# Chunyu-Hugh/SymbolicRegression.jl

Hardware: AMD Instinct MI355X
Metric: tree-node x row evals/sec (batched eval_loss, fp32) (higher is better)
Workload: dtype f32

## Files before the change

symbolicregression.jl_amd/csrc/sr_capi.cpp:

```cpp
#include <hip/hip_runtime.h>
#include <rccl/rccl.h>
#include <dlfcn.h>
#include <limits.h>
#include <stdlib.h>

#include <algorithm>
#include <atomic>
#include <chrono>
#include <cmath>
#include <cstdio>
#include <cstdlib>
#include <cstring>
#include <deque>
#include <functional>
#include <memory>
#include <mutex>
#include <string>
#include <vector>

#include "../../include/sr_amd.h"
#include "sr_compile.h"
#include "sr_eval.h"
#include "sr_fold.h"
#include "sr_fold_dev.h"
// ... 864 lines not shown
    prog->max_depth = 0;
    prog->tier = tier;
    prog->max_checks = 0;
    prog->total_nodes = 0;
    prog->total_ops = 0;
    hprog = ctx->h_prog.as<char>();
    h_code = reinterpret_cast<SrIns<T>*>(hprog);
    h_off = reinterpret_cast<uint32_t*>(hprog + img.o_off);
    h_bad = reinterpret_cast<uint8_t*>(hprog + img.o_bad);
    h_perm = reinterpret_cast<uint32_t*>(hprog + img.o_perm);
    ctx->h_bad_last = h_bad;
    ctx->h_perm_last = h_perm;
    h_end = reinterpret_cast<uint32_t*>(hprog + img.o_end);
    last.n_chunks = 0;
    last.derived = false;
    last.n_derived = 0;
    last.timed = ctx->timing != 0 && !want.internal;
    if (last.timed) SR_HIP_CHECK(hipEventRecord(ctx->ev_start, s));
    if (gather)
      SR_HIP_CHECK(hipMemcpyAsync(ctx->row_idx.p, req.row_idx, size_t(n_rows_up) * sizeof(int64_t), hipMemcpyHostToDevice,
                                  s));
    if (parametric && nt > 0 && p_stride > 0)
      SR_HIP_CHECK(hipMemcpyAsync(ctx->ptab.p, ctx->h_ptab.p, size_t(nt) * size_t(p_stride) * sizeof(T), hipMemcpyHostToDevice, s));
    return SR_OK;
  }

  int launch_derived() {
    dld = (n_eval + kRowAlign - 1) / kRowAlign * kRowAlign;
    max_abs_x = leaf_bound(want.shard ? want.shard->max_abs_x : req.ds->max_abs_x);
    const int64_t derived_rows = want.shard ? want.shard->min_rows : n_eval;
    if (allow_derived && ctx->derived && want.mode == SR_MODE_LOSS && tier == SR_TIER_BASIC &&
        derived_rows >= kDerivedMinRows && nt >= 64 && double(nt) * double(derived_rows) >= kDerivedMinWork &&
        max_abs_x < double(tbig())) {
      choose_derived(*req.trees, ctx->opsets[req.opset_id], req.ds->nf, &spec, &dmap);
      if (spec.n > 0) {
        SR_HIP_CHECK(ctx->derived_cols.ensure(size_t(spec.n) * size_t(dld) * sizeof(T)));
        if (last.timed) SR_HIP_CHECK(hipEventRecord(ctx->ev_d0, s));
        SR_HIP_CHECK(sr_launch_derived<T>(static_cast<const T*>(req.ds->X), req.ds->ld,
                                          gather ? ctx->row_idx.as<int64_t>() : nullptr, n_eval, dld, spec,
                                          ctx->derived_cols.as<T>(), dld, s));
        if (last.timed) SR_HIP_CHECK(hipEventRecord(ctx->ev_d1, s));
        last.derived = true;
        last.n_derived = spec.n;
      } else {
        dmap.clear();
      }
    }
    stress_probe = use_probe && !gather && req.ds->probe_rows != nullptr && ctx->stress_probe;
    if (stress_probe && !dmap.empty()) {
      SR_HIP_CHECK(ctx->probe_derived.ensure(size_t(spec.n) * size_t(kProbeRows) * sizeof(T)));
      SR_HIP_CHECK(sr_launch_derived<T>(static_cast<const T*>(req.ds->X), req.ds->ld,
                                        static_cast<const int64_t*>(req.ds->probe_rows), req.ds->n_probe, kProbeRows, spec,
                                        ctx->probe_derived.as<T>(), kProbeRows, s));
    }
    return SR_OK;
  }

  int begin_chunks() {
    if (n_chunks > 1) {
      SR_HIP_CHECK(ctx->need_stream2());
      SR_HIP_CHECK(hipEventRecord(ctx->ev_join, s));
      SR_HIP_CHECK(hipStreamWaitEvent(ctx->stream2, ctx->ev_join, 0));
    }
    fjob.path = fold.path;
    fjob.tier = tier;
    fjob.gather = gather;
    fjob.n_eval = n_eval;
// ... 3452 lines not shown
```

symbolicregression.jl_amd/csrc/sr_compile.cpp:

```cpp
#include "sr_compile.h"

#include <unistd.h>

#include <algorithm>
#include <atomic>
#include <chrono>
#include <cstdlib>
#include <cmath>
#include <condition_variable>
#include <cstring>
#include <functional>
#include <mutex>
#include <thread>

namespace {

class WorkerPool {
 public:
  static WorkerPool& get() {
    static std::mutex m;
    static WorkerPool* pool = nullptr;
    std::lock_guard<std::mutex> g(m);
    if (!pool || pool->pid_ != getpid()) pool = new WorkerPool();
    return *pool;
// ... 129 lines not shown
  std::vector<T> fold_val;
  std::vector<int32_t> const_slot;
  std::vector<int32_t> need;
  std::vector<SrIns<T>> code;
  std::vector<int32_t> sz;
  bool bad = false;
  int err = SR_OK;
  std::string msg;
  int depth = 0, max_depth = 0;
  uint32_t n_checks = 0;
  uint32_t n_consts = 0;
  int64_t n_ops = 0;

  const int16_t* derived = nullptr;
  int max_params = 0;
  const bool fuse_pbc = [] {
    static const bool on = [] {
      const char* v = std::getenv("SR_AMD_PBC");
      return !(v && v[0] == '0');
    }();
    return on;
  }();

  TreeCompiler(const SrOpset& o, int64_t nr, int64_t nf, bool wci, const int16_t* dm = nullptr)
      : ops(o), n_rows(nr), nfeatures(nf), with_const_index(wci), derived(dm) {}

  int derived_col(int i) {
    if (!derived || t.degree[i] != 1) return -1;
    const int c = t.l[i];
    if (t.degree[c] != 0 || t.constant[c] || par(c)) return -1;
    const uint32_t u = unary_id(i);
    if (u == SR_U_NONE || u >= SR_U_COUNT) return -1;
    return derived[size_t(u) * size_t(nfeatures) + size_t(t.feature[c] - 1)];
  }

  bool leaf(int i) const { return t.degree[i] == 0; }
  bool par(int i) const { return t.is_param != nullptr && t.is_param[i] != 0; }
  bool effleaf(int i) const { return t.degree[i] == 0 || folded[i]; }

  uint32_t unary_id(int i) {
    const int k = int(t.op[i]) - 1;
    if (k < 0 || k >= int(ops.unary.size())) {
      fail(SR_ERR_BAD_TREE, "unary op index out of range");
      return SR_U_NONE;
    }
    return ops.unary[k];
  }
  uint32_t binary_id(int i) {
    const int k = int(t.op[i]) - 1;
    if (k < 0 || k >= int(ops.binary.size())) {
      fail(SR_ERR_BAD_TREE, "binary op index out of range");
      return SR_B_NONE;
    }
    return ops.binary[k];
  }
  void fail(int code, const char* m) {
    if (err == SR_OK) {
      err = code;
      msg = m;
    }
  }

  bool parse() {
    const int64_t n = t.n;
    if (n <= 0) {
      fail(SR_ERR_BAD_TREE, "empty tree");
// ... 270 lines not shown
    const bool free_c = base == SR_OP_LOAD_FEAT || base == SR_OP_LOAD_FEAT_PUSH ||
                        (base >= SR_OP_UNARY0 && base < SR_OP_LOAD_DERIVED) ||
                        (base >= SR_OP_BINARY0 && base < SR_OP_LOAD_PARAM && (base - SR_OP_BINARY0) % 6u < SR_V_CL) ||
                        (base >= SR_OP_LOAD_PARAM && base < SR_OP_PAIR0);
    if (!free_c) return false;
    uint32_t v = 0;
    switch (bop) {
      case SR_B_ADD: v = SR_PBC_ADD; break;
      case SR_B_SUB: v = left ? SR_PBC_SUB_L : SR_PBC_SUB_R; break;
      case SR_B_MUL: v = SR_PBC_MUL; break;
      case SR_B_DIV: v = left ? SR_PBC_DIV_L : SR_PBC_DIV_R; break;
      default: return false;
    }
    const_operand_check(leaf);
    last.op |= v << SR_OP_PBC_SHIFT;
    last.c0 = lf.c0;
    last.c1 = lf.c1;
    if (arr_check[i]) {
      last.op |= SR_OP_PBC_CHECK;
      ++n_checks;
    }
    return true;
  }

  void emit(int i) {
    if (effleaf(i)) {
      code.push_back(leaf_ins(i));
      emit_check(i);
      return;
    }
    const int d = t.degree[i];
    ++n_ops;
    if (d == 1) {
      const int dc = infsub[i] ? -1 : derived_col(i);
      if (dc >= 0) {
        SrIns<T> in{};
        in.op = SR_OP_LOAD_DERIVED;
        in.meta = uint32_t(dc);
        in.c0 = (unary_id(i) << 16) | uint32_t(t.feature[t.l[i]] - 1);
        code.push_back(in);
        emit_check(i);
        return;
      }
      emit(t.l[i]);
      if (!with_const_index && !code.empty() && (code.back().op >> SR_OP_POST_SHIFT) == 0u) {
        code.back().op |= (unary_id(i) << SR_OP_POST_SHIFT) | (infsub[i] ? SR_OP_POST_INF : 0u);
        if (arr_check[i]) {
          code.back().op |= SR_OP_POST_CHECK;
          ++n_checks;
        }
        return;
      }
      SrIns<T> in{};
      in.op = (infsub[i] ? SR_OP_UNARY_INF0 : SR_OP_UNARY0) + unary_id(i);
      code.push_back(in);
      emit_check(i);
      return;
    }
    const int a = t.l[i], b = t.r[i];
    const uint32_t bop = binary_id(i);
    if (err != SR_OK) return;
    if (emit_pair(i, bop)) {
    } else if (effleaf(b) && !(!with_const_index && par(b) && effleaf(a) && !par(a))) {
      emit(a);
      if (fuse_const_operand(i, b, bop, false)) return;
      const_operand_check(b);
// ... 294 lines not shown
```

symbolicregression.jl_amd/csrc/sr_compile.h:

```cpp
#pragma once
#include <stdint.h>
#include <functional>
#include <string>
#include <vector>
#include "sr_ops.h"
#include "../../include/sr_amd.h"

struct SrOpset {
  std::vector<uint32_t> unary;
  std::vector<uint32_t> binary;
};

uint32_t sr_unary_id(const char* name);
uint32_t sr_binary_id(const char* name);

template <typename T>
struct SrProgramBatch {
  std::vector<SrIns<T>> code;
  std::vector<uint32_t> offsets;
  std::vector<uint8_t> static_bad;
  std::vector<uint32_t> n_checks;
  std::vector<uint32_t> n_consts;
  std::vector<uint32_t> const_off;
  std::vector<uint32_t> cost;
  std::vector<uint8_t> depth;
  int max_depth = 0;
  int tier = 1;
  int max_checks = 0;
  int64_t total_nodes = 0;
  int64_t total_ops = 0;
  bool keep_pieces = false;
  std::vector<std::vector<SrIns<T>>> pieces;
  std::vector<uint32_t> piece, begin;
  size_t n_code = 0;
  const SrIns<T>* tree_code(size_t k) const {
    return keep_pieces ? pieces[piece[k]].data() + begin[k] : code.data() + offsets[k];
  }
};

void sr_parallel_for(int n, const std::function<void(int)>& fn);

uint32_t sr_instruction_cost(uint32_t opcode);

struct SrParamNodes {
  const uint8_t* is_parameter;
  const uint16_t* parameter;
  int32_t max_parameters;
};
template <typename T>
int sr_compile_batch(const sr_tree_batch& trees, const SrOpset& ops, int64_t n_rows, int64_t nfeatures,
                     bool with_const_index, SrProgramBatch<T>* out, std::string* err,
                     const int16_t* derived = nullptr, const SrParamNodes* pn = nullptr);
```

symbolicregression.jl_amd/csrc/sr_knobs.h:

```cpp
#pragma once
#include <stdint.h>
#include <stdlib.h>
#include <string.h>

#include <string>

#include "sr_plan.h"

struct SrKnobs {
  int tail_chunk = 4;
  int exact_early = 1;
  int64_t fold_seg = -1;
  int64_t host_reduce = 8192;
  int host_io = 1;
  int debug_hint_regrow = 0;
  int exact_g = 0;
  int exact_w = 4;
  int derived = 1;
  int stress_probe = 1;
  int code_cache = 1;
  int vstk_rows = 0;
  int grad_rows_force = 0;
  int grad_sort = 1;
  int grad_lane_bins = 1;
  int first_chunk = 6;
  int64_t chunk_min = 1024;
  int inject_fail = 0;
  int inject_post = 0;
  int inject_post_exact = 0;
  int inject_post_gather = 0;
  int inject_post_wsum = 0;
  int timing = 1;
  int rows_override = 0;
  int tree_group = 0;
  int waves_override = 0;
  bool cost_order = true;
  bool balance_groups = true;
  bool dead_hints = true;
  int max_row_blocks = 512;
  int chunks = 2;
  int probe = 2;
  int ref_fold = 1;
  int64_t fold_store_mb = 512;
  int64_t fold_slot_mb = 24576;
  int fold_delta_log2 = 8;
  int64_t fold_seg_max = 16384;
  int64_t fold_rows_max = int64_t(1) << 24;
  int fold_debug_fail = 0;
  int fold_single_pass = 1;
  int fold_compact = 1;
  int64_t fold_list_wgs = 2048;
// ... 9 lines not shown
struct SrKnobRow {
  const char* name;
  const char* env;
  int SrKnobs::*i32;
  int64_t SrKnobs::*i64;
  bool SrKnobs::*flag;
  SrKnobNorm norm;
  int64_t lo, hi;
  const char* refuse;
  bool env_inverse;

  constexpr SrKnobRow(const char* n, const char* e, int SrKnobs::*m, SrKnobNorm nm = SR_KNOB_RANGE, int64_t l = INT64_MIN,
                      int64_t h = INT64_MAX, const char* r = nullptr)
      : name(n), env(e), i32(m), i64(nullptr), flag(nullptr), norm(nm), lo(l), hi(h), refuse(r), env_inverse(false) {}
  constexpr SrKnobRow(const char* n, const char* e, int64_t SrKnobs::*m, int64_t l = INT64_MIN, int64_t h = INT64_MAX)
      : name(n), env(e), i32(nullptr), i64(m), flag(nullptr), norm(SR_KNOB_RANGE), lo(l), hi(h), refuse(nullptr),
        env_inverse(false) {}
  constexpr SrKnobRow(const char* n, const char* e, bool SrKnobs::*m, bool inverse = false)
      : name(n), env(e), i32(nullptr), i64(nullptr), flag(m), norm(SR_KNOB_FLAG), lo(0), hi(1), refuse(nullptr),
        env_inverse(inverse) {}
};

constexpr int64_t kKnobMax = INT64_MAX;

constexpr SrKnobRow kSrKnobs[] = {
    {"rows_per_lane", "SR_AMD_ROWS_PER_LANE", &SrKnobs::rows_override},
    {"trees_per_block", "SR_AMD_TREES_PER_BLOCK", &SrKnobs::tree_group, SR_KNOB_RANGE, 0, 256,
     "trees_per_block: 0, or 1..256 (4 waves of 64 slots)"},
    {nullptr, "SR_AMD_WAVES", &SrKnobs::waves_override},
    {"vstk_rows", "SR_AMD_VSTK_ROWS", &SrKnobs::vstk_rows},
    {"max_row_blocks", "SR_AMD_MAX_ROW_BLOCKS", &SrKnobs::max_row_blocks, SR_KNOB_RANGE, 1, 1 << 16},
    {"code_cache", "SR_AMD_CODE_CACHE", &SrKnobs::code_cache, SR_KNOB_FLAG},
    {"derived", "SR_AMD_DERIVED", &SrKnobs::derived, SR_KNOB_FLAG},
    {nullptr, "SR_AMD_NO_SORT", &SrKnobs::cost_order, true},
    {"balance", "SR_AMD_BALANCE", &SrKnobs::balance_groups},
    {nullptr, "SR_AMD_NO_HINT", &SrKnobs::dead_hints, true},
    {"probe", "SR_AMD_PROBE", &SrKnobs::probe},
    {"stress_probe", "SR_AMD_STRESS_PROBE", &SrKnobs::stress_probe, SR_KNOB_FLAG},
    {nullptr, "SR_AMD_CHUNKS", &SrKnobs::chunks},
    {"first_chunk", "SR_AMD_FIRST_CHUNK", &SrKnobs::first_chunk, SR_KNOB_RANGE, 2, 64},
    {"chunk_min", "SR_AMD_CHUNK_MIN", &SrKnobs::chunk_min, 1, kKnobMax},
    {"tail_chunk", "SR_AMD_TAIL_CHUNK", &SrKnobs::tail_chunk, SR_KNOB_RANGE, 0, kTailTwelfths,
     "tail_chunk: 0, or the last chunk's twelfths 1..6"},
    {"host_io", "SR_AMD_HOST_IO", &SrKnobs::host_io, SR_KNOB_RANGE, 0, 1, "host_io must be 0 or 1"},
    {"host_reduce", "SR_AMD_HOST_REDUCE", &SrKnobs::host_reduce, 0, kKnobMax},
    {"timing", nullptr, &SrKnobs::timing, SR_KNOB_FLAG},
    {"exact_g", "SR_AMD_EXACT_G", &SrKnobs::exact_g, SR_KNOB_RANGE, 0, 64},
    {"exact_w", "SR_AMD_EXACT_W", &SrKnobs::exact_w, SR_KNOB_EXACT_W},
    {"exact_early", "SR_AMD_EXACT_EARLY", &SrKnobs::exact_early, SR_KNOB_FLAG},
    {"grad_rows", "SR_AMD_GRAD_ROWS", &SrKnobs::grad_rows_force},
    {"grad_sort", "SR_AMD_GRAD_SORT", &SrKnobs::grad_sort, SR_KNOB_FLAG},
    {"grad_lane_bins", nullptr, &SrKnobs::grad_lane_bins, SR_KNOB_FLAG},
    {"ref_fold", "SR_AMD_REF_FOLD", &SrKnobs::ref_fold, SR_KNOB_FLAG},
    {"fold_seg", "SR_AMD_FOLD_SEG", &SrKnobs::fold_seg, -1, kKnobMax},
    {"fold_store_mb", "SR_AMD_FOLD_STORE_MB", &SrKnobs::fold_store_mb, 0, kKnobMax},
    {"fold_slot_mb", "SR_AMD_FOLD_SLOT_MB", &SrKnobs::fold_slot_mb, 1, kKnobMax},
    {"fold_delta_log2", "SR_AMD_FOLD_DELTA_LOG2", &SrKnobs::fold_delta_log2, SR_KNOB_RANGE, 1, 40},
    {"fold_seg_max", "SR_AMD_FOLD_SEG_MAX", &SrKnobs::fold_seg_max, 0, kKnobMax},
    {"fold_rows_max", "SR_AMD_FOLD_ROWS_MAX", &SrKnobs::fold_rows_max, 0, kKnobMax},
    {"fold_single_pass", "SR_AMD_FOLD_SINGLE_PASS", &SrKnobs::fold_single_pass, SR_KNOB_FLAG},
    {"fold_compact", "SR_AMD_FOLD_COMPACT", &SrKnobs::fold_compact, SR_KNOB_FLAG},
    {"fold_list_wgs", "SR_AMD_FOLD_LIST_WGS", &SrKnobs::fold_list_wgs, 0, kFoldListWgsMax},
    {"loss_compact", "SR_AMD_LOSS_COMPACT", &SrKnobs::loss_compact, SR_KNOB_FLAG},
    {"loss_list_groups", "SR_AMD_LOSS_LIST_GROUPS", &SrKnobs::loss_list_groups, SR_KNOB_RANGE, 0, 1 << 20},
    {"fold_cand_est", "SR_AMD_FOLD_CAND_EST", &SrKnobs::fold_cand_est, SR_KNOB_FLAG},
    {"fold_cand_est_min", "SR_AMD_FOLD_CAND_EST_MIN", &SrKnobs::fold_cand_est_min, SR_KNOB_RANGE, 1, 1 << 30},
// ... 43 lines not shown
```

symbolicregression.jl_amd/csrc/sr_plan.h:

```cpp
#pragma once
#include <stddef.h>
#include <stdint.h>

#include <algorithm>
#include <utility>
#include <vector>

#include "sr_compile.h"
#include "../../include/sr_amd.h"

enum { SR_MODE_LOSS = 0, SR_MODE_PRED = 1, SR_MODE_EXACT = 2, SR_MODE_FOLD = 3 };
#ifndef SR_VSTK_SLOTS
#define SR_VSTK_SLOTS 2
#endif
enum { SR_TIER_BASIC = 0, SR_TIER_FULL = 1 };
enum { SR_TIER_PARAM = 2 };
enum { SR_TIER_CAND = 4 };

struct SrSegment {
  int block0, pos0, n_pos, groups;
  int64_t row_off;
};

constexpr int SR_MAX_DERIVED = 32;
struct SrDerivedSpec {
  int n;
  uint8_t op[SR_MAX_DERIVED];
  uint16_t feat[SR_MAX_DERIVED];
};

template <typename T>
inline int sr_rows_per_lane(int mode, int tier, int requested) {
  const bool basic = mode == SR_MODE_LOSS && tier == SR_TIER_BASIC;
  if (sizeof(T) == 4) {
    if (basic) return (requested == 4 || requested == 16) ? requested : 8;
    return 4;
  }
  return basic ? 4 : 2;
}

inline size_t sr_tile_lds_bytes(int elem_size, int nf, int rows_per_lane, int stack_depth, int trees_per_block,
                                int max_checks, int waves, bool weighted, int code_lds = 0) {
  const size_t rows = size_t(64) * rows_per_lane;
  return size_t(nf) * rows * elem_size + (weighted ? 2 : 1) * rows * elem_size +
         size_t(waves) * stack_depth * rows * elem_size + size_t(waves) * size_t(max_checks) * rows * elem_size +
         (size_t(trees_per_block) * size_t(max_checks) * elem_size + 15) / 16 * 16 + size_t(code_lds) * 16;
}

inline int sr_waves_per_block(int elem_size, int mode, int tier, int rows_per_lane, int requested) {
  if (elem_size == 4 && mode == SR_MODE_LOSS && tier == SR_TIER_BASIC && rows_per_lane == 8 && requested == 8)
    return 8;
  return 4;
}

#ifndef SR_VSTK_DEFAULT_ROWS
#define SR_VSTK_DEFAULT_ROWS 16
#endif
inline int sr_vstk_rows(int elem_size, int64_t n_rows, int requested) {
  if (elem_size == 8) {
    if (requested == 8 || requested == -4) return requested == 8 ? 8 : 4;
// ... 91 lines not shown
      p.n = 3;
      p.bound[1] = first;
      p.bound[2] = nt - last;
      p.bound[3] = nt;
      return p;
    }
  }
  p.n = sr_chunk_count(nt, chunks, first_chunk, chunk_min, multi, mode);
  for (int k = 0; k <= p.n; ++k) p.bound[k] = sr_chunk_bound(k, p.n, nt, first_chunk);
  return p;
}

inline size_t sr_align256(size_t x) { return (x + 255) & ~size_t(255); }
struct ProgImage {
  size_t code_cap = 0;
  size_t o_off = 0, o_bad = 0, o_perm = 0, o_end = 0, o_seg = 0, bytes = 0;
};
inline ProgImage sr_prog_image(int64_t total_nodes, int64_t nt, size_t ins_size, size_t n_seg_cap) {
  ProgImage m;
  m.code_cap = size_t(total_nodes) + 16;
  m.o_off = sr_align256(m.code_cap * ins_size);
  m.o_bad = sr_align256(m.o_off + (size_t(nt) + 1) * sizeof(uint32_t));
  m.o_perm = sr_align256(m.o_bad + size_t(nt) + 16);
  m.o_end = sr_align256(m.o_perm + (size_t(nt) + 1) * sizeof(uint32_t));
  m.o_seg = sr_align256(m.o_end + (size_t(nt) + 1) * sizeof(uint32_t));
  m.bytes = m.o_seg + n_seg_cap * sizeof(SrSegment);
  return m;
}

constexpr int64_t kDerivedMinRows = 16384;
constexpr int kDerivedMinUses = 4;
constexpr double kDerivedMinWork = 33554432.0;
constexpr int64_t kDerivedSample = 1024;
inline void choose_derived(const sr_tree_batch& trees, const SrOpset& ops, int64_t nf, SrDerivedSpec* spec,
                           std::vector<int16_t>* dmap) {
  spec->n = 0;
  dmap->assign(size_t(SR_U_COUNT) * size_t(nf), int16_t(-1));
  auto eligible = [](uint32_t u) {
    return u == SR_U_EXP || u == SR_U_COS || u == SR_U_SIN || u == SR_U_LOG || u == SR_U_SQRT;
  };
  std::vector<int32_t> uses(size_t(SR_U_COUNT) * size_t(nf), 0);
  const int64_t ns = trees.n_trees < kDerivedSample ? trees.n_trees : kDerivedSample;
  for (int64_t k = 0; k < ns; ++k) {
    const int64_t b = trees.offsets[k], e = trees.offsets[k + 1];
    for (int64_t i = b; i + 1 < e; ++i) {
      if (trees.degree[i] != 1 || trees.degree[i + 1] != 0 || trees.constant[i + 1]) continue;
      const int oi = int(trees.op[i]) - 1;
      const int f = int(trees.feature[i + 1]) - 1;
      if (oi < 0 || oi >= int(ops.unary.size()) || f < 0 || f >= nf) continue;
      const uint32_t u = ops.unary[size_t(oi)];
      if (eligible(u)) ++uses[size_t(u) * size_t(nf) + size_t(f)];
    }
  }
  std::vector<std::pair<int32_t, size_t>> cand;
  for (size_t q = 0; q < uses.size(); ++q)
    if (uses[q] >= kDerivedMinUses) cand.push_back({uses[q], q});
  std::stable_sort(cand.begin(), cand.end(), [](const auto& x, const auto& y) { return x.first > y.first; });
  for (const auto& c : cand) {
    if (spec->n >= SR_MAX_DERIVED) break;
    const int k = spec->n++;
    spec->op[k] = uint8_t(c.second / size_t(nf));
    spec->feat[k] = uint16_t(c.second % size_t(nf));
    (*dmap)[c.second] = int16_t(k);
  }
}

inline int64_t sr_count_vstk(const uint8_t* depth, int64_t nc, bool vstk) {
  int64_t n_vs = 0;
  if (vstk)
    for (int64_t i = 0; i < nc; ++i) n_vs += depth[i] <= SR_VSTK_SLOTS ? 1 : 0;
  return n_vs;
}
inline void sr_cost_sort(const uint32_t* cost, const uint8_t* depth, int64_t nc, const int32_t* tree_view, int n_views,
                         bool sort, bool vstk, uint32_t* perm) {
  uint32_t cmax = 0;
  if (sort)
    for (int64_t i = 0; i < nc; ++i) cmax = cost[i] > cmax ? cost[i] : cmax;
  const size_t nkey = size_t(cmax) + 1;
  const size_t n_cls = tree_view ? size_t(n_views) : 2;
  std::vector<uint32_t> start(n_cls * nkey + 1, 0);
  auto key = [&](int64_t i) -> size_t {
    const size_t cls = tree_view ? size_t(tree_view[i]) : ((vstk && depth[i] > SR_VSTK_SLOTS) ? 1 : 0);
    return cls * nkey + (sort ? size_t(cmax - cost[i]) : 0);
  };
  for (int64_t i = 0; i < nc; ++i) ++start[key(i) + 1];
  for (size_t k = 1; k < start.size(); ++k) start[k] += start[k - 1];
  for (int64_t i = 0; i < nc; ++i) perm[start[key(i)]++] = uint32_t(i);
}
inline void sr_deal_groups(uint32_t* perm, int64_t np, int64_t G, int64_t ng) {
  if (np <= 1 || ng <= 1) return;
  std::vector<uint32_t> ranked(perm, perm + np);
  int64_t k = 0;
  for (int64_t j = 0; j < G; ++j)
    for (int64_t gi = 0; gi < ng; ++gi) {
      const int64_t size = gi + 1 < ng ? G : np - (ng - 1) * G;
      if (j < size) perm[gi * G + j] = ranked[size_t(k++)];
// ... 126 lines not shown
```

symbolicregression.jl_amd/csrc/sr_tile_impl.h:

```cpp
#include <hip/hip_runtime.h>
#include <stdint.h>

#include <type_traits>

#include "sr_eval.h"
#include "sr_fold_dev.h"
#include "sr_ops.h"

template <int W>
struct SrMinWaves {
  static constexpr int value = W >= 16 ? 8 : (W >= 8 ? 6 : 1);
};
#ifndef SR_MIN_WAVES_W4
#define SR_MIN_WAVES_W4 5
#endif
#ifndef SR_MIN_WAVES_R16
#define SR_MIN_WAVES_R16 2
#endif
#ifndef SR_MIN_WAVES_VSTK16
#define SR_MIN_WAVES_VSTK16 4
#endif

#ifndef SR_MIN_WAVES_VSTK8
#define SR_MIN_WAVES_VSTK8 6
// ... 344 lines not shown
__device__ __forceinline__ void sr_unary_rows(T (&v)[R]) {
  if constexpr (sizeof(T) == 4 && ID == SR_U_EXP && R % 2 == 0) {
    sr_exp_rows_f32<R>(v);
  } else if constexpr (sizeof(T) == 4 && (ID == SR_U_LOG || ID == SR_U_COS || ID == SR_U_SIN)) {
    SrRowVec<R> x;
#pragma unroll
    for (int r = 0; r < R; ++r) x[r] = v[r];
    bool slow = false;
    if constexpr (ID == SR_U_COS || ID == SR_U_SIN) {
      float m = 0.0f;
#pragma unroll
      for (int r = 0; r + 1 < R; r += 2) m = SrMaxAbs<float>::step(m, v[r], v[r + 1]);
      if constexpr (R % 2 != 0) m = SrMaxAbs<float>::step(m, v[R - 1], v[R - 1]);
      slow = !(m < srl::kTrigFastLimit);
    }
    if constexpr (ID == SR_U_LOG)
      x = sr_log_rows<R>(x);
    else if (__builtin_amdgcn_ballot_w64(slow) == 0)
      x = sr_trig_rows_fast<ID, R>(x);
    else
      x = sr_libm_rows<ID, R>(x);
#pragma unroll
    for (int r = 0; r < R; ++r) v[r] = x[r];
  } else if constexpr (sizeof(T) == 8 && (ID == SR_U_EXP || ID == SR_U_LOG || ID == SR_U_COS || ID == SR_U_SIN)) {
    SrRowVecD<ID, R> x;
#pragma unroll
    for (int r = 0; r < R; ++r) x[r] = v[r];
    x = sr_libm_rows_f64<ID, R>(x);
#pragma unroll
    for (int r = 0; r < R; ++r) v[r] = x[r];
  } else {
#pragma unroll
    for (int r = 0; r < R; ++r) v[r] = sr_unary<T>(ID, v[r]);
  }
}

#define SR_POST_CASE(ID) \
  case ID:               \
    sr_unary_rows<T, ID, R>(tos); \
    break;
template <typename T, int R, int TIER, bool FAST>
__device__ __forceinline__ void sr_post_unary(uint32_t u, bool inf, T (&tos)[R]) {
  uint32_t nonfin = 0u;
  if constexpr (!FAST) {
    if (inf) {
#pragma unroll
      for (int r = 0; r < R; ++r) nonfin |= sr_isfinite(tos[r]) ? 0u : (1u << r);
    }
  }
  switch (u) {
    SR_POST_CASE(SR_U_NEG) SR_POST_CASE(SR_U_SQUARE) SR_POST_CASE(SR_U_CUBE) SR_POST_CASE(SR_U_EXP)
    SR_POST_CASE(SR_U_COS) SR_POST_CASE(SR_U_SIN) SR_POST_CASE(SR_U_LOG) SR_POST_CASE(SR_U_SQRT)
    SR_POST_CASE(SR_U_ABS)
    default:
      if constexpr (TIER == SR_TIER_FULL) {
        switch (u) {
          SR_POST_CASE(SR_U_TAN) SR_POST_CASE(SR_U_LOG2) SR_POST_CASE(SR_U_LOG10) SR_POST_CASE(SR_U_LOG1P)
          SR_POST_CASE(SR_U_SIGN) SR_POST_CASE(SR_U_TANH) SR_POST_CASE(SR_U_SINH) SR_POST_CASE(SR_U_COSH)
          SR_POST_CASE(SR_U_ATAN) SR_POST_CASE(SR_U_ASIN) SR_POST_CASE(SR_U_ACOS) SR_POST_CASE(SR_U_ACOSH)
          SR_POST_CASE(SR_U_ATANH) SR_POST_CASE(SR_U_ASINH) SR_POST_CASE(SR_U_RELU) SR_POST_CASE(SR_U_INV)
          SR_POST_CASE(SR_U_ERF) SR_POST_CASE(SR_U_ERFC) SR_POST_CASE(SR_U_GAMMA) SR_POST_CASE(SR_U_ROUND)
          SR_POST_CASE(SR_U_FLOOR) SR_POST_CASE(SR_U_CEIL) SR_POST_CASE(SR_U_EXP2) SR_POST_CASE(SR_U_EXPM1)
          default: break;
        }
      }
      break;
// ... 602 lines not shown
              SR_PUSH_TOS();
              [[fallthrough]];
            case SR_OP_LOAD_FEAT: {
              L::load(SR_OPND_X(), tos);
              if (FAST_CHECK && a.track_x && (SR_META() & SR_M_CHECK)) {
                SR_TRACK();
              }
              break;
            }
            case SR_OP_LOAD_PARAM_PUSH:
              if constexpr (PARAM) {
                SR_PUSH_TOS();
              }
              [[fallthrough]];
            case SR_OP_LOAD_PARAM: {
              if constexpr (PARAM) {
                SR_PARAM_ROWS(tos);
                if (FAST_CHECK && a.track_x && (SR_META() & SR_M_CHECK)) {
                  SR_TRACK();
                }
              }
              break;
            }
            case SR_OP_LOAD_DERIVED_PUSH:
              SR_PUSH_TOS();
              [[fallthrough]];
            case SR_OP_LOAD_DERIVED: {
              if constexpr (FAST_CHECK) {
                L::load(a.derived + size_t(SR_META() & SR_M_INDEX) * size_t(a.dld) + size_t(row0) + size_t(lane * C), tos);
                SR_TRACK();
              } else {
                const uint32_t uf = uint32_t(__builtin_amdgcn_readlane(int(wc0), int(k)));
                L::load(sr_row_at<ROWS>(x_lane, uf & 0xffffu), tos);
                switch (uf >> 16) {
                  case SR_U_EXP: sr_unary_rows<T, SR_U_EXP, R>(tos); break;
                  case SR_U_COS: sr_unary_rows<T, SR_U_COS, R>(tos); break;
                  case SR_U_SIN: sr_unary_rows<T, SR_U_SIN, R>(tos); break;
                  case SR_U_LOG: sr_unary_rows<T, SR_U_LOG, R>(tos); break;
                  case SR_U_SQRT: sr_unary_rows<T, SR_U_SQRT, R>(tos); break;
                  default: break;
                }
              }
              break;
            }
            case SR_OP_LOAD_CONST_PUSH:
              SR_PUSH_TOS();
              [[fallthrough]];
            case SR_OP_LOAD_CONST: {
              const T cv = SR_CVAL();
#pragma unroll
              for (int r = 0; r < R; ++r) tos[r] = cv;
              SR_TRACK();
              break;
            }
            SR_UCASE(SR_U_NEG) SR_UCASE(SR_U_SQUARE) SR_UCASE(SR_U_CUBE) SR_UCASE(SR_U_EXP)
            SR_UCASE(SR_U_COS) SR_UCASE(SR_U_SIN) SR_UCASE(SR_U_LOG) SR_UCASE(SR_U_SQRT)
            SR_UCASE(SR_U_ABS)
            SR_BCASE_COMM(SR_B_ADD) SR_BCASE_COMM(SR_B_MUL) SR_BCASE(SR_B_SUB) SR_BCASE(SR_B_DIV)
            SR_UCASE_FULL(SR_U_TAN) SR_UCASE_FULL(SR_U_LOG2) SR_UCASE_FULL(SR_U_LOG10)
            SR_UCASE_FULL(SR_U_LOG1P) SR_UCASE_FULL(SR_U_SIGN) SR_UCASE_FULL(SR_U_TANH)
            SR_UCASE_FULL(SR_U_SINH) SR_UCASE_FULL(SR_U_COSH) SR_UCASE_FULL(SR_U_ATAN)
            SR_UCASE_FULL(SR_U_ASIN) SR_UCASE_FULL(SR_U_ACOS) SR_UCASE_FULL(SR_U_ACOSH)
            SR_UCASE_FULL(SR_U_ATANH) SR_UCASE_FULL(SR_U_ASINH) SR_UCASE_FULL(SR_U_RELU)
            SR_UCASE_FULL(SR_U_INV) SR_UCASE_FULL(SR_U_ERF) SR_UCASE_FULL(SR_U_ERFC)
            SR_UCASE_FULL(SR_U_GAMMA) SR_UCASE_FULL(SR_U_ROUND) SR_UCASE_FULL(SR_U_FLOOR)
            SR_UCASE_FULL(SR_U_CEIL) SR_UCASE_FULL(SR_U_EXP2) SR_UCASE_FULL(SR_U_EXPM1)
            SR_BCASE_FULL(SR_B_POW) SR_BCASE_FULL(SR_B_MAX) SR_BCASE_FULL(SR_B_MIN)
            SR_BCASE_FULL(SR_B_MOD) SR_BCASE_FULL(SR_B_GREATER) SR_BCASE_FULL(SR_B_LESS)
            SR_BCASE_FULL(SR_B_GREATER_EQUAL) SR_BCASE_FULL(SR_B_LESS_EQUAL) SR_BCASE_FULL(SR_B_COND)
            SR_BCASE_FULL(SR_B_LOGICAL_OR) SR_BCASE_FULL(SR_B_LOGICAL_AND) SR_BCASE_FULL(SR_B_ATAN2)
            SR_BCASE_PR(SR_B_ADD, true) SR_BCASE_PR(SR_B_MUL, true) SR_BCASE_P(SR_B_SUB, true)
            SR_BCASE_P(SR_B_DIV, true)
            SR_BCASE_P(SR_B_POW, TIER == SR_TIER_FULL) SR_BCASE_P(SR_B_MAX, TIER == SR_TIER_FULL)
// ... 302 lines not shown
                 (((emask >> lane) & 1u) ? SR_FLAG_ELEMINF : 0u);
    if (MODE == SR_MODE_LOSS && a.out_sum) {
      const uint32_t tree = a.perm ? a.perm[my_pos] : uint32_t(my_pos);
      if (a.static_bad[tree]) f |= SR_FLAG_STATIC | SR_FLAG_NONFINITE;
      a.out_sum[tree] = accv;
      a.out_flag[tree] = f;
    } else {
      const size_t o = size_t(rb) * a.n_trees + my_pos;
      a.part_sum[o] = accv;
      a.part_flag[o] = f;
    }
  }
  SR_STAMP(6);
}

template <typename T, int R, int MODE, bool GATHER, int TIER, int W, int LK, bool VSTK>
hipError_t sr_launch_tile(const SrEvalArgs<T>& a, int n_blocks, hipStream_t s) {
  if (VSTK && a.stack_depth > SR_VSTK_SLOTS) return hipErrorInvalidValue;
  if constexpr ((TIER & SR_TIER_PARAM) != 0) {
    if (a.ptab == nullptr || a.n_classes < 1 || a.p_stride < 0 || a.nf < 2) return hipErrorInvalidValue;
  }
  const SrLdsPlan<T> plan(a.nf, 64 * R, VSTK ? 0 : a.stack_depth, a.trees_per_block,
                          MODE == SR_MODE_EXACT ? a.max_checks : 0, W, a.w != nullptr,
                          (MODE == SR_MODE_LOSS || MODE == SR_MODE_FOLD) ? a.code_lds : 0);
  const void* fn = reinterpret_cast<const void*>(&sr_tile_kernel<T, R, MODE, GATHER, TIER, W, LK, VSTK>);
  if (plan.total > 65536) {
    const hipError_t e = hipFuncSetAttribute(fn, hipFuncAttributeMaxDynamicSharedMemorySize, int(plan.total));
    if (e != hipSuccess) return e;
  }
  hipLaunchKernelGGL((sr_tile_kernel<T, R, MODE, GATHER, TIER, W, LK, VSTK>), dim3(n_blocks), dim3(W * 64), plan.total, s, a);
  return hipGetLastError();
}

template <typename T, int R>
__global__ void __launch_bounds__(256) sr_derived_kernel(const T* __restrict__ X, int64_t ld, const int64_t* row_idx,
                                                         int64_t n_view, int64_t n_pad, SrDerivedSpec spec,
                                                         T* __restrict__ out, int64_t dld) {
  sr_libm_lds_fill(int(threadIdx.x), 256);
  __syncthreads();
  const int k = int(blockIdx.y);
  const int64_t v0 = (int64_t(blockIdx.x) * 256 + threadIdx.x) * R;
  if (v0 >= n_pad) return;
  const T* xf = X + int64_t(spec.feat[k]) * ld;
  T v[R];
#pragma unroll
  for (int r = 0; r < R; ++r) {
    const int64_t q = v0 + r;
    v[r] = xf[row_idx ? row_idx[q < n_view ? q : 0] : q];
  }
  switch (spec.op[k]) {
    case SR_U_EXP: sr_unary_rows<T, SR_U_EXP, R>(v); break;
    case SR_U_COS: sr_unary_rows<T, SR_U_COS, R>(v); break;
    case SR_U_SIN: sr_unary_rows<T, SR_U_SIN, R>(v); break;
    case SR_U_LOG: sr_unary_rows<T, SR_U_LOG, R>(v); break;
    case SR_U_SQRT: sr_unary_rows<T, SR_U_SQRT, R>(v); break;
    default: break;
  }
  T* o = out + size_t(k) * size_t(dld) + size_t(v0);
#pragma unroll
  for (int r = 0; r < R; ++r) o[r] = v[r];
}

template <typename T>
hipError_t sr_launch_derived(const T* X, int64_t ld, const int64_t* row_idx, int64_t n_view, int64_t n_pad,
                             const SrDerivedSpec& spec, T* out, int64_t dld, hipStream_t s) {
  constexpr int R = 8;
  if (spec.n <= 0) return hipSuccess;
  const int64_t per_block = 256 * R;
  const dim3 grid(unsigned((n_pad + per_block - 1) / per_block), unsigned(spec.n));
  hipLaunchKernelGGL((sr_derived_kernel<T, R>), grid, dim3(256), 0, s, X, ld, row_idx, n_view, n_pad, spec, out, dld);
  return hipGetLastError();
}
```

Measured before the change: 31880 billion.

## Add chained unary derived columns and per-feature fused derived kernel

Adds optional precomputed columns for nested unary pairs such as sin(exp(x)). These are selected by sampled use counts and gated by a new knob that is off by default. The derived-column kernel is restructured to group columns per feature. It loads each feature tile once with vectorized loads, computes each inner op once, and writes plain and chained outputs using a grid-stride loop with 16-byte stores. The intent is to cut redundant feature reads and repeated transcendental evaluations in the precompute pass. The cost is a larger derived map, extra branching in the tile kernel's derived-load path, and a new alignment requirement.

Result: no change. 31770 billion (-0.3%).

```diff
diff --git a/symbolicregression.jl_amd/csrc/sr_capi.cpp b/symbolicregression.jl_amd/csrc/sr_capi.cpp
--- a/symbolicregression.jl_amd/csrc/sr_capi.cpp
+++ b/symbolicregression.jl_amd/csrc/sr_capi.cpp
@@ -920,7 +920,12 @@
     if (allow_derived && ctx->derived && want.mode == SR_MODE_LOSS && tier == SR_TIER_BASIC &&
         derived_rows >= kDerivedMinRows && nt >= 64 && double(nt) * double(derived_rows) >= kDerivedMinWork &&
         max_abs_x < double(tbig())) {
-      choose_derived(*req.trees, ctx->opsets[req.opset_id], req.ds->nf, &spec, &dmap);
+      SrDerivedRule rule;
+      rule.chain_min_uses = ctx->derived_chain ? ctx->derived_chain_min : 0;
+      rule.max_abs_x = max_abs_x;
+      rule.tbig = double(tbig());
+      rule.col_bytes = dld * int64_t(sizeof(T));
+      choose_derived(*req.trees, ctx->opsets[req.opset_id], req.ds->nf, &spec, &dmap, rule);
       if (spec.n > 0) {
         SR_HIP_CHECK(ctx->derived_cols.ensure(size_t(spec.n) * size_t(dld) * sizeof(T)));
         if (last.timed) SR_HIP_CHECK(hipEventRecord(ctx->ev_d0, s));
diff --git a/symbolicregression.jl_amd/csrc/sr_compile.cpp b/symbolicregression.jl_amd/csrc/sr_compile.cpp
--- a/symbolicregression.jl_amd/csrc/sr_compile.cpp
+++ b/symbolicregression.jl_amd/csrc/sr_compile.cpp
@@ -185,6 +185,18 @@
     const uint32_t u = unary_id(i);
     if (u == SR_U_NONE || u >= SR_U_COUNT) return -1;
     return derived[size_t(u) * size_t(nfeatures) + size_t(t.feature[c] - 1)];
+  }
+
+  int chain_col(int i, uint32_t* inner) {
+    if (!derived || t.degree[i] != 1 || !infsub[i]) return -1;
+    const int c = t.l[i];
+    if (t.degree[c] != 1) return -1;
+    const int g = t.l[c];
+    if (t.degree[g] != 0 || t.constant[g] || par(g)) return -1;
+    const int so = sr_derived_op_slot(unary_id(i)), si = sr_derived_op_slot(unary_id(c));
+    if (so < 0 || si < 0) return -1;
+    *inner = unary_id(c);
+    return derived[sr_derived_chain_index(so, si, nfeatures, t.feature[g] - 1)];
   }
 
   bool leaf(int i) const { return t.degree[i] == 0; }
@@ -521,6 +533,17 @@
     const int d = t.degree[i];
     ++n_ops;
     if (d == 1) {
+      uint32_t inner = SR_U_NONE;
+      const int cc = chain_col(i, &inner);
+      if (cc >= 0) {
+        SrIns<T> in{};
+        in.op = SR_OP_LOAD_DERIVED;
+        in.meta = uint32_t(cc);
+        in.c0 = (inner << 24) | (unary_id(i) << 16) | uint32_t(t.feature[t.l[t.l[i]]] - 1);
+        code.push_back(in);
+        emit_check(i);
+        return;
+      }
       const int dc = infsub[i] ? -1 : derived_col(i);
       if (dc >= 0) {
         SrIns<T> in{};
diff --git a/symbolicregression.jl_amd/csrc/sr_compile.h b/symbolicregression.jl_amd/csrc/sr_compile.h
--- a/symbolicregression.jl_amd/csrc/sr_compile.h
+++ b/symbolicregression.jl_amd/csrc/sr_compile.h
@@ -42,6 +42,23 @@
 
 uint32_t sr_instruction_cost(uint32_t opcode);
 
+constexpr int kDerivedOps = 5;
+inline int sr_derived_op_slot(uint32_t u) {
+  switch (u) {
+    case SR_U_EXP: return 0;
+    case SR_U_COS: return 1;
+    case SR_U_SIN: return 2;
+    case SR_U_LOG: return 3;
+    case SR_U_SQRT: return 4;
+    default: return -1;
+  }
+}
+inline size_t sr_derived_map_size(int64_t nf) {
+  return (size_t(SR_U_COUNT) + size_t(kDerivedOps) * kDerivedOps) * size_t(nf);
+}
+inline size_t sr_derived_chain_index(int outer_slot, int inner_slot, int64_t nf, int64_t f) {
+  return size_t(SR_U_COUNT) * size_t(nf) + (size_t(outer_slot) * kDerivedOps + size_t(inner_slot)) * size_t(nf) + size_t(f);
+}
 struct SrParamNodes {
   const uint8_t* is_parameter;
   const uint16_t* parameter;
diff --git a/symbolicregression.jl_amd/csrc/sr_knobs.h b/symbolicregression.jl_amd/csrc/sr_knobs.h
--- a/symbolicregression.jl_amd/csrc/sr_knobs.h
+++ b/symbolicregression.jl_amd/csrc/sr_knobs.h
@@ -17,6 +17,8 @@
   int exact_g = 0;
   int exact_w = 4;
   int derived = 1;
+  int derived_chain = 0;
+  int derived_chain_min = kDerivedChainMinUses;
   int stress_probe = 1;
   int code_cache = 1;
   int vstk_rows = 0;
@@ -92,6 +94,8 @@
     {"max_row_blocks", "SR_AMD_MAX_ROW_BLOCKS", &SrKnobs::max_row_blocks, SR_KNOB_RANGE, 1, 1 << 16},
     {"code_cache", "SR_AMD_CODE_CACHE", &SrKnobs::code_cache, SR_KNOB_FLAG},
     {"derived", "SR_AMD_DERIVED", &SrKnobs::derived, SR_KNOB_FLAG},
+    {"derived_chain", "SR_AMD_DERIVED_CHAIN", &SrKnobs::derived_chain, SR_KNOB_FLAG},
+    {"derived_chain_min", "SR_AMD_DERIVED_CHAIN_MIN", &SrKnobs::derived_chain_min, SR_KNOB_RANGE, 1, 1 << 20},
     {nullptr, "SR_AMD_NO_SORT", &SrKnobs::cost_order, true},
     {"balance", "SR_AMD_BALANCE", &SrKnobs::balance_groups},
     {nullptr, "SR_AMD_NO_HINT", &SrKnobs::dead_hints, true},
diff --git a/symbolicregression.jl_amd/csrc/sr_plan.h b/symbolicregression.jl_amd/csrc/sr_plan.h
--- a/symbolicregression.jl_amd/csrc/sr_plan.h
+++ b/symbolicregression.jl_amd/csrc/sr_plan.h
@@ -3,6 +3,7 @@
 #include <stdint.h>
 
 #include <algorithm>
+#include <cmath>
 #include <utility>
 #include <vector>
 
@@ -22,10 +23,12 @@
   int64_t row_off;
 };
 
-constexpr int SR_MAX_DERIVED = 32;
+constexpr int SR_MAX_DERIVED = 64;
+constexpr int SR_MAX_DERIVED_PLAIN = 32;
 struct SrDerivedSpec {
   int n;
   uint8_t op[SR_MAX_DERIVED];
+  uint8_t inner[SR_MAX_DERIVED];
   uint16_t feat[SR_MAX_DERIVED];
 };
 
@@ -183,24 +186,50 @@
 constexpr int kDerivedMinUses = 4;
 constexpr double kDerivedMinWork = 33554432.0;
 constexpr int64_t kDerivedSample = 1024;
+constexpr int64_t kDerivedMaxBytes = int64_t(1) << 30;
+constexpr int kDerivedChainMinUses = 4;
+inline bool sr_derived_inner_ok(uint32_t v, double max_abs_x, double tbig) {
+  if (!(max_abs_x < tbig)) return false;
+  switch (v) {
+    case SR_U_COS: case SR_U_SIN: return 1.0 < tbig;
+    case SR_U_LOG: return 745.2 < tbig && max_abs_x < tbig;
+    case SR_U_SQRT: return 1.0 < tbig;
+    case SR_U_EXP: return tbig > 0.0 && max_abs_x < std::log(tbig) - 1e-3;
+    default: return false;
+  }
+}
+struct SrDerivedRule {
+  int chain_min_uses = 0;
+  double max_abs_x = 0.0;
+  double tbig = 0.0;
+  int64_t col_bytes = 0;
+};
 inline void choose_derived(const sr_tree_batch& trees, const SrOpset& ops, int64_t nf, SrDerivedSpec* spec,
-                           std::vector<int16_t>* dmap) {
+                           std::vector<int16_t>* dmap, const SrDerivedRule& rule = SrDerivedRule()) {
   spec->n = 0;
-  dmap->assign(size_t(SR_U_COUNT) * size_t(nf), int16_t(-1));
-  auto eligible = [](uint32_t u) {
-    return u == SR_U_EXP || u == SR_U_COS || u == SR_U_SIN || u == SR_U_LOG || u == SR_U_SQRT;
+  dmap->assign(sr_derived_map_size(nf), int16_t(-1));
+  auto eligible = [](uint32_t u) { return sr_derived_op_slot(u) >= 0; };
+  auto unary_of = [&](int64_t i) -> uint32_t {
+    const int oi = int(trees.op[i]) - 1;
+    return (oi < 0 || oi >= int(ops.unary.size())) ? uint32_t(SR_U_NONE) : ops.unary[size_t(oi)];
   };
   std::vector<int32_t> uses(size_t(SR_U_COUNT) * size_t(nf), 0);
+  std::vector<int32_t> chain_uses(size_t(kDerivedOps) * kDerivedOps * size_t(nf), 0);
   const int64_t ns = trees.n_trees < kDerivedSample ? trees.n_trees : kDerivedSample;
   for (int64_t k = 0; k < ns; ++k) {
     const int64_t b = trees.offsets[k], e = trees.offsets[k + 1];
     for (int64_t i = b; i + 1 < e; ++i) {
       if (trees.degree[i] != 1 || trees.degree[i + 1] != 0 || trees.constant[i + 1]) continue;
-      const int oi = int(trees.op[i]) - 1;
       const int f = int(trees.feature[i + 1]) - 1;
-      if (oi < 0 || oi >= int(ops.unary.size()) || f < 0 || f >= nf) continue;
-      const uint32_t u = ops.unary[size_t(oi)];
-      if (eligible(u)) ++uses[size_t(u) * size_t(nf) + size_t(f)];
+      const uint32_t u = unary_of(i);
+      if (u == SR_U_NONE || f < 0 || f >= nf) continue;
+      if (!eligible(u)) continue;
+      ++uses[size_t(u) * size_t(nf) + size_t(f)];
+      if (rule.chain_min_uses > 0 && i > b && trees.degree[i - 1] == 1) {
+        const uint32_t o = unary_of(i - 1);
+        if (eligible(o))
+          ++chain_uses[(size_t(sr_derived_op_slot(o)) * kDerivedOps + size_t(sr_derived_op_slot(u))) * size_t(nf) + size_t(f)];
+      }
     }
   }
   std::vector<std::pair<int32_t, size_t>> cand;
@@ -208,11 +237,30 @@
     if (uses[q] >= kDerivedMinUses) cand.push_back({uses[q], q});
   std::stable_sort(cand.begin(), cand.end(), [](const auto& x, const auto& y) { return x.first > y.first; });
   for (const auto& c : cand) {
-    if (spec->n >= SR_MAX_DERIVED) break;
+    if (spec->n >= SR_MAX_DERIVED_PLAIN) break;
     const int k = spec->n++;
     spec->op[k] = uint8_t(c.second / size_t(nf));
+    spec->inner[k] = uint8_t(SR_U_NONE);
     spec->feat[k] = uint16_t(c.second % size_t(nf));
     (*dmap)[c.second] = int16_t(k);
+  }
+  if (rule.chain_min_uses <= 0) return;
+  static const uint32_t kOps[kDerivedOps] = {SR_U_EXP, SR_U_COS, SR_U_SIN, SR_U_LOG, SR_U_SQRT};
+  cand.clear();
+  for (size_t q = 0; q < chain_uses.size(); ++q) {
+    const uint32_t inner = kOps[(q / size_t(nf)) % kDerivedOps];
+    if (chain_uses[q] >= rule.chain_min_uses && sr_derived_inner_ok(inner, rule.max_abs_x, rule.tbig))
+      cand.push_back({chain_uses[q], q});
+  }
+  std::stable_sort(cand.begin(), cand.end(), [](const auto& x, const auto& y) { return x.first > y.first; });
+  for (const auto& c : cand) {
+    if (spec->n >= SR_MAX_DERIVED) break;
+    if (rule.col_bytes > 0 && int64_t(spec->n + 1) > kDerivedMaxBytes / rule.col_bytes) break;
+    const int k = spec->n++;
+    spec->op[k] = uint8_t(kOps[c.second / (size_t(nf) * kDerivedOps)]);
+    spec->inner[k] = uint8_t(kOps[(c.second / size_t(nf)) % kDerivedOps]);
+    spec->feat[k] = uint16_t(c.second % size_t(nf));
+    (*dmap)[size_t(SR_U_COUNT) * size_t(nf) + c.second] = int16_t(k);
   }
 }
 
diff --git a/symbolicregression.jl_amd/csrc/sr_tile_impl.h b/symbolicregression.jl_amd/csrc/sr_tile_impl.h
--- a/symbolicregression.jl_amd/csrc/sr_tile_impl.h
+++ b/symbolicregression.jl_amd/csrc/sr_tile_impl.h
@@ -400,6 +400,18 @@
   } else {
 #pragma unroll
     for (int r = 0; r < R; ++r) v[r] = sr_unary<T>(ID, v[r]);
+  }
+}
+
+template <typename T, int R>
+__device__ __forceinline__ void sr_derived_rows(uint32_t u, T (&v)[R]) {
+  switch (u) {
+    case SR_U_EXP: sr_unary_rows<T, SR_U_EXP, R>(v); break;
+    case SR_U_COS: sr_unary_rows<T, SR_U_COS, R>(v); break;
+    case SR_U_SIN: sr_unary_rows<T, SR_U_SIN, R>(v); break;
+    case SR_U_LOG: sr_unary_rows<T, SR_U_LOG, R>(v); break;
+    case SR_U_SQRT: sr_unary_rows<T, SR_U_SQRT, R>(v); break;
+    default: break;
   }
 }
 
@@ -1068,13 +1080,18 @@
               } else {
                 const uint32_t uf = uint32_t(__builtin_amdgcn_readlane(int(wc0), int(k)));
                 L::load(sr_row_at<ROWS>(x_lane, uf & 0xffffu), tos);
-                switch (uf >> 16) {
-                  case SR_U_EXP: sr_unary_rows<T, SR_U_EXP, R>(tos); break;
-                  case SR_U_COS: sr_unary_rows<T, SR_U_COS, R>(tos); break;
-                  case SR_U_SIN: sr_unary_rows<T, SR_U_SIN, R>(tos); break;
-                  case SR_U_LOG: sr_unary_rows<T, SR_U_LOG, R>(tos); break;
-                  case SR_U_SQRT: sr_unary_rows<T, SR_U_SQRT, R>(tos); break;
-                  default: break;
+                constexpr bool kChains = (TIER & SR_TIER_FULL) == 0;
+                const uint32_t inner = kChains ? (uf >> 24) : 0u;
+                if (inner != 0u) sr_derived_rows<T, R>(inner, tos);
+                uint32_t nonfin = 0u;
+                if (inner != 0u) {
+#pragma unroll
+                  for (int r = 0; r < R; ++r) nonfin |= sr_isfinite(tos[r]) ? 0u : (1u << r);
+                }
+                sr_derived_rows<T, R>(kChains ? ((uf >> 16) & 0xffu) : (uf >> 16), tos);
+                if (inner != 0u) {
+#pragma unroll
+                  for (int r = 0; r < R; ++r) tos[r] = ((nonfin >> r) & 1u) ? sr_inf<T>() : tos[r];
                 }
               }
               break;
@@ -1443,42 +1460,130 @@
   return hipGetLastError();
 }
 
-template <typename T, int R>
+
+struct SrDerivedFeat {
+  uint16_t feat;
+  uint8_t need;
+  int8_t plain[kDerivedOps];
+  int8_t chain[kDerivedOps][kDerivedOps];
+};
+constexpr int kDerivedFeatsPerLaunch = 16;
+constexpr int kDerivedTileRows = 2048;
+struct SrDerivedPass {
+  int n;
+  SrDerivedFeat f[kDerivedFeatsPerLaunch];
+};
+static_assert(SR_MAX_DERIVED <= 128, "SrDerivedFeat holds column numbers in int8_t");
+
+__device__ __forceinline__ uint32_t sr_derived_slot_op(int slot) {
+  switch (slot) {
+    case 0: return SR_U_EXP;
+    case 1: return SR_U_COS;
+    case 2: return SR_U_SIN;
+    case 3: return SR_U_LOG;
+    default: return SR_U_SQRT;
+  }
+}
+
+template <typename T, bool VEC>
 __global__ void __launch_bounds__(256) sr_derived_kernel(const T* __restrict__ X, int64_t ld, const int64_t* row_idx,
-                                                         int64_t n_view, int64_t n_pad, SrDerivedSpec spec,
+                                                         int64_t n_view, int64_t n_pad, SrDerivedPass pass,
                                                          T* __restrict__ out, int64_t dld) {
+  constexpr int R = 8, V = 16 / int(sizeof(T)), NV = R / V;
+  typedef T vec_t __attribute__((ext_vector_type(V)));
+  static_assert(256 * R == kDerivedTileRows, "tile rows");
   sr_libm_lds_fill(int(threadIdx.x), 256);
   __syncthreads();
-  const int k = int(blockIdx.y);
-  const int64_t v0 = (int64_t(blockIdx.x) * 256 + threadIdx.x) * R;
-  if (v0 >= n_pad) return;
-  const T* xf = X + int64_t(spec.feat[k]) * ld;
-  T v[R];
-#pragma unroll
-  for (int r = 0; r < R; ++r) {
-    const int64_t q = v0 + r;
-    v[r] = xf[row_idx ? row_idx[q < n_view ? q : 0] : q];
-  }
-  switch (spec.op[k]) {
-    case SR_U_EXP: sr_unary_rows<T, SR_U_EXP, R>(v); break;
-    case SR_U_COS: sr_unary_rows<T, SR_U_COS, R>(v); break;
-    case SR_U_SIN: sr_unary_rows<T, SR_U_SIN, R>(v); break;
-    case SR_U_LOG: sr_unary_rows<T, SR_U_LOG, R>(v); break;
-    case SR_U_SQRT: sr_unary_rows<T, SR_U_SQRT, R>(v); break;
-    default: break;
-  }
-  T* o = out + size_t(k) * size_t(dld) + size_t(v0);
-#pragma unroll
-  for (int r = 0; r < R; ++r) o[r] = v[r];
+  const SrDerivedFeat& pf = pass.f[blockIdx.y];
+  const T* xf = X + int64_t(pf.feat) * ld;
+  const int64_t n_tiles = n_pad / kDerivedTileRows;
+  auto store = [&](int col, int64_t base, const T(&v)[R]) {
+    T* o = out + size_t(col) * size_t(dld) + size_t(base);
+#pragma unroll
+    for (int j = 0; j < NV; ++j) {
+      vec_t w;
+#pragma unroll
+      for (int e = 0; e < V; ++e) w[e] = v[j * V + e];
+      *reinterpret_cast<vec_t*>(o + (j * 256 + int(threadIdx.x)) * V) = w;
+    }
+  };
+  for (int64_t tile = blockIdx.x; tile < n_tiles; tile += gridDim.x) {
+    const int64_t base = tile * kDerivedTileRows;
+    T x[R];
+#pragma unroll
+    for (int j = 0; j < NV; ++j) {
+      const int64_t q = base + (j * 256 + int(threadIdx.x)) * V;
+      if constexpr (VEC) {
+        const vec_t w = *reinterpret_cast<const vec_t*>(xf + q);
+#pragma unroll
+        for (int e = 0; e < V; ++e) x[j * V + e] = w[e];
+      } else {
+#pragma unroll
+        for (int e = 0; e < V; ++e) {
+          const int64_t qq = q + e;
+          x[j * V + e] = xf[row_idx ? row_idx[qq < n_view ? qq : 0] : qq];
+        }
+      }
+    }
+    for (int vi = 0; vi < kDerivedOps; ++vi) {
+      if (((pf.need >> vi) & 1u) == 0u) continue;
+      T v[R];
+#pragma unroll
+      for (int r = 0; r < R; ++r) v[r] = x[r];
+      sr_derived_rows<T, R>(sr_derived_slot_op(vi), v);
+      if (pf.plain[vi] >= 0) store(pf.plain[vi], base, v);
+      for (int ui = 0; ui < kDerivedOps; ++ui) {
+        const int col = pf.chain[vi][ui];
+        if (col < 0) continue;
+        T w[R];
+#pragma unroll
+        for (int r = 0; r < R; ++r) w[r] = v[r];
+        sr_derived_rows<T, R>(sr_derived_slot_op(ui), w);
+        store(col, base, w);
+      }
+    }
+  }
 }
 
 template <typename T>
 hipError_t sr_launch_derived(const T* X, int64_t ld, const int64_t* row_idx, int64_t n_view, int64_t n_pad,
                              const SrDerivedSpec& spec, T* out, int64_t dld, hipStream_t s) {
-  constexpr int R = 8;
   if (spec.n <= 0) return hipSuccess;
-  const int64_t per_block = 256 * R;
-  const dim3 grid(unsigned((n_pad + per_block - 1) / per_block), unsigned(spec.n));
-  hipLaunchKernelGGL((sr_derived_kernel<T, R>), grid, dim3(256), 0, s, X, ld, row_idx, n_view, n_pad, spec, out, dld);
-  return hipGetLastError();
-}
+  if (spec.n > SR_MAX_DERIVED || n_pad % kDerivedTileRows != 0 || dld < n_pad) return hipErrorInvalidValue;
+  std::vector<SrDerivedFeat> feats;
+  for (int k = 0; k < spec.n; ++k) {
+    size_t i = 0;
+    while (i < feats.size() && feats[i].feat != spec.feat[k]) ++i;
+    if (i == feats.size()) {
+      SrDerivedFeat nf{};
+      nf.feat = spec.feat[k];
+      for (int v = 0; v < kDerivedOps; ++v) {
+        nf.plain[v] = -1;
+        for (int u = 0; u < kDerivedOps; ++u) nf.chain[v][u] = -1;
+      }
+      feats.push_back(nf);
+    }
+    const int so = sr_derived_op_slot(spec.op[k]);
+    const int si = spec.inner[k] ? sr_derived_op_slot(spec.inner[k]) : so;
+    if (so < 0 || si < 0) return hipErrorInvalidValue;
+    if (spec.inner[k]) feats[i].chain[si][so] = int8_t(k);
+    else feats[i].plain[so] = int8_t(k);
+    feats[i].need |= uint8_t(1u << si);
+  }
+  const int64_t n_tiles = n_pad / kDerivedTileRows;
+  const bool vec = row_idx == nullptr && reinterpret_cast<uintptr_t>(X) % 16 == 0 && (size_t(ld) * sizeof(T)) % 16 == 0;
+  if (reinterpret_cast<uintptr_t>(out) % 16 != 0 || (size_t(dld) * sizeof(T)) % 16 != 0) return hipErrorInvalidValue;
+  for (size_t f0 = 0; f0 < feats.size(); f0 += kDerivedFeatsPerLaunch) {
+    SrDerivedPass pass{};
+    pass.n = int(std::min<size_t>(kDerivedFeatsPerLaunch, feats.size() - f0));
+    for (int i = 0; i < pass.n; ++i) pass.f[i] = feats[f0 + size_t(i)];
+    const dim3 grid(unsigned(std::min<int64_t>(n_tiles, 256)), unsigned(pass.n));
+    if (vec)
+      hipLaunchKernelGGL((sr_derived_kernel<T, true>), grid, dim3(256), 0, s, X, ld, row_idx, n_view, n_pad, pass, out, dld);
+    else
+      hipLaunchKernelGGL((sr_derived_kernel<T, false>), grid, dim3(256), 0, s, X, ld, row_idx, n_view, n_pad, pass, out, dld);
+    const hipError_t e = hipGetLastError();
+    if (e != hipSuccess) return e;
+  }
+  return hipSuccess;
+}
```
